# mengxuyiGit/LGM

Measured on AMD Instinct MI355X. Metric: Mpixels/s fwd+bwd Gaussian raster (256^2, 100k gauss, 6 views), higher is better.
Workload: dtype f32

## Files before the change

lgm_amd/csrc/render_common.h:

```cpp
#pragma once
#include <hip/hip_runtime.h>
#include <stdint.h>

#include "common.h"
#include "lgm_render.h"
#include "work_split.h"

namespace lgm {

constexpr int BX = 16, BY = 16, TILE_PIX = BX * BY;
constexpr int NACC = 10;
constexpr int NACC_V = 6, NACC_S = 4;
__host__ __device__ __forceinline__ size_t acc_index(int q, size_t bvN_i, size_t bN_i, size_t BVN) {
    return q < 5 ? bvN_i * NACC_V + q : q < 9 ? BVN * NACC_V + bN_i * NACC_S + (q - 5) : bvN_i * NACC_V + 5;
}
__host__ __device__ inline size_t acc_elems(size_t B, size_t V, size_t N) { return B * V * N * NACC_V + B * N * NACC_S; }
__host__ __device__ inline size_t acc_side_offset(size_t B, size_t V, size_t N) { return (acc_elems(B, V, N) + 1) & ~(size_t)1; }
__host__ __device__ inline int det_flush_limit_log2(int V, int T, bool scene_record) {
    const long long f = scene_record ? (long long)V * T : (long long)T;
    int c = 0;
    while ((1ll << c) < f) c++;
    return 62 - c;
}
constexpr int LDS_HIST_MAX = 8192;
// ... 214 lines not shown
    const float pw = 1.0f / (hom[3] + 0.0000001f);
    const float ppx = hom[0] * pw, ppy = hom[1] * pw;
    xf43(Vw, g[0], g[1], g[2], pv);
    if (pv[2] <= 0.2f) return false;
    const ProjCtx P = make_proj(Vw, g[0], g[1], g[2], d.fx, d.fy, d.tanx, d.tany);
    float a, b, c;
    cov2d(P, c3, a, b, c);
    const float det = a * c - b * b;
    if (det == 0.0f) return false;
    const float det_inv = 1.f / det;
    const float mid = 0.5f * (a + c);
    const float l1 = mid + sqrtf(fmaxf(0.1f, mid * mid - det));
    const float l2 = mid - sqrtf(fmaxf(0.1f, mid * mid - det));
    const float rad = ceilf(3.f * sqrtf(fmaxf(l1, l2)));
    const float px = ndc2pix(ppx, d.W), py = ndc2pix(ppy, d.H);
    const int r = (int)rad;
    const int x0 = min(d.gx, max(0, (int)((px - r) / BX)));
    const int y0 = min(d.gy, max(0, (int)((py - r) / BY)));
    const int x1 = min(d.gx, max(0, (int)((px + r + BX - 1) / BX)));
    const int y1 = min(d.gy, max(0, (int)((py + r + BY - 1) / BY)));
    if ((x1 - x0) * (y1 - y0) == 0) return false;
    o.x = px; o.y = py; o.depth = pv[2];
    o.A = c * det_inv; o.B = -b * det_inv; o.C = a * det_inv;
    o.opacity = g[3];
    o.x0 = x0; o.y0 = y0; o.x1 = x1; o.y1 = y1; o.radius = r;
    const float op = g[3];
    if (d.options & LGM_RENDER_NO_CULL) {
        o.hx = o.hy = 3.0e38f;
        o.tau = 3.0e38f;
        o.cx0 = x0; o.cx1 = x1; o.cy0 = y0; o.cy1 = y1;
        return true;
    }
    if (!(op * 255.0f > 1.0f)) {
        o.hx = o.hy = -1.f;
        o.tau = -1.f;
        o.cx0 = o.cx1 = x0; o.cy0 = o.cy1 = y0;
        return true;
    }
    const float cond = (a + c) * (a + c) * __builtin_amdgcn_rcpf(det);
    if (!(det > 0.f) || !(cond < 4e4f)) {
        o.hx = o.hy = 3.0e38f;
        o.tau = 3.0e38f;
        o.cx0 = x0; o.cx1 = x1; o.cy0 = y0; o.cy1 = y1;
        return true;
    }
    const float tau = (2.0f * 0.6931471805599453f) * __builtin_amdgcn_logf(255.0f * op) * (1.001f + 2e-5f * cond) + 1e-3f;
    o.tau = tau;
    o.hx = sqrtf(tau * fmaxf(a, 0.f));
    o.hy = sqrtf(tau * fmaxf(c, 0.f));
    const float lx = fmaxf(-1.0f, fminf((float)d.gx, (px - o.hx - (BX - 1)) / BX));
    const float hxt = fmaxf(-1.0f, fminf((float)d.gx, (px + o.hx) / BX));
    const float ly = fmaxf(-1.0f, fminf((float)d.gy, (py - o.hy - (BY - 1)) / BY));
    const float hyt = fmaxf(-1.0f, fminf((float)d.gy, (py + o.hy) / BY));
    o.cx0 = max(x0, (int)ceilf(lx));
    o.cx1 = min(x1, (int)floorf(hxt) + 1);
    o.cy0 = max(y0, (int)ceilf(ly));
    o.cy1 = min(y1, (int)floorf(hyt) + 1);
    if (o.cx1 < o.cx0) o.cx1 = o.cx0;
    if (o.cy1 < o.cy0) o.cy1 = o.cy0;
    return true;
}

__device__ __forceinline__ void load_gaussian(const float *__restrict__ src, float g[14]) {
    const float2 *p = reinterpret_cast<const float2 *>(src);
#pragma unroll
    for (int k = 0; k < 7; k++) {
        const float2 v = p[k];
        g[2 * k] = v.x;
        g[2 * k + 1] = v.y;
    }
}

__device__ __forceinline__ void tile_range(int tile, long long slot_stride, const int *__restrict__ tile_start,
                                           const int *__restrict__ tile_count, long long &base, int &n) {
    if (slot_stride >= 0) {
        base = (long long)tile * slot_stride;
        n = tile_count[tile];
    } else {
        base = tile_start[tile];
        n = tile_start[tile + 1] - tile_start[tile];
    }
}

__host__ __device__ __forceinline__ int round8(int x) { return (x + 7) & ~7; }

__device__ __forceinline__ void tile_pixel(int t, int &lx, int &ly) {
    const int w = t >> 6, l = t & 63;
    lx = ((w & 1) << 3) + (l & 7);
    ly = ((w >> 1) << 3) + (l >> 3);
}

int launch_binning(const Dims &d, const float *gaussians, const float *cam_view, const float *cam_view_proj,
                   char *ws, const Layout &L, int *radii_out, long long *stats_out, bool count_only,
                   hipStream_t st);
int launch_render_fwd(const Dims &d, const float *gaussians, const float *bg, float *image, float *depth,
                      float *alpha, char *ws, const Layout &L, hipStream_t st);
int launch_loss_reduce(const Dims &d, char *ws, const Layout &L, hipStream_t st);
int launch_render_bwd(const Dims &d, const float *gaussians, const float *cam_view, const float *cam_view_proj,
                      const float *bg, const float *d_image, const float *d_depth, const float *d_alpha,
                      float *d_gaussians, float *d_means2D, char *ws, const Layout &L, hipStream_t st);

}
```

lgm_amd/csrc/render_raster.hip:

```cpp
#include "cdna4.h"
#include "render_common.h"

#include <type_traits>

namespace lgm {
namespace {

__device__ __forceinline__ unsigned long long lanemask_lt(int lane) { return (1ull << lane) - 1ull; }

#if defined(LGM_BWD_STAMPS) || defined(LGM_FWD_STAMPS)
__device__ __forceinline__ unsigned long long sec_stamp() {
    unsigned long long t;
    __builtin_amdgcn_sched_barrier(0);
    asm volatile("s_memtime %0\n\ts_waitcnt lgkmcnt(0)" : "=s"(t)::"memory");
    __builtin_amdgcn_sched_barrier(0);
    return t;
}
#define SEC_T(v) const unsigned long long v = sec_stamp()
#define SEC_ADD(acc, a, b) acc += (b) - (a)
#else
#define SEC_T(v)
#define SEC_ADD(acc, a, b)
#endif

// ... 121 lines not shown
                                                    const unsigned long long *__restrict__ pairs,
                                                    const float4 *__restrict__ gP, const float4 *__restrict__ gQ,
                                                    const float *__restrict__ gauss,
                                                    const float *__restrict__ bg, float *__restrict__ out_img,
                                                    float *__restrict__ out_depth, float *__restrict__ out_alpha,
                                                    float *__restrict__ final_T, int *__restrict__ n_contrib,
                                                    int *__restrict__ wlast_out,
                                                    unsigned char *__restrict__ cmask, float4 *__restrict__ cfin,
                                                    float *__restrict__ ck, int2 *__restrict__ cklist,
                                                    int *__restrict__ nck, unsigned *__restrict__ ckctr,
                                                    int ck_region, float4 *__restrict__ zero_base,
                                                    long long zero_n16) {
    __shared__ StageT<1, FU> S;
    __shared__ int s_ck[2];
    const int tile = xcd_item(blockIdx.x, d.BV * d.T);
    const int bv = tile / d.T, t = tile - bv * d.T, b = bv / d.V;
    const int tx0 = (t % d.gx) * BX, ty0 = (t / d.gx) * BY;
    const int tid = threadIdx.x, w = tid >> 6, lane = tid & 63;
    int lx, ly;
    tile_pixel(tid, lx, ly);
    const int px = tx0 + lx, py = ty0 + ly;
    const bool inside = px < d.W && py < d.H;
    const float pfx = (float)px, pfy = (float)py;
    long long base;
    int n;
    tile_range(tile, slot_stride, tile_start, tile_count, base, n);
    const unsigned *ids = reinterpret_cast<const unsigned *>(pairs + base);
    const size_t gbase = (size_t)bv * d.N;
    const unsigned long long t_start = __builtin_amdgcn_s_memrealtime();
    init_sentinel(S);
    float Tr = inside ? 1.0f : -1.0f, C0 = 0.f, C1 = 0.f, C2 = 0.f, D = 0.f;
    int last = 0;
    unsigned c_iter = 0, c_list = 0;
    unsigned id_a = tid < n ? ids[tid] : 0u;
    unsigned id_b = TILE_PIX + tid < n ? ids[TILE_PIX + tid] : 0u;
    const int ck_reg = xcd_group(tile, d.BV * d.T);
    const bool det_ck = (d.options & LGM_RENDER_DETERMINISTIC) != 0;
    int ck_slot = -1, ck_written = 0;
#ifdef LGM_FWD_STAMPS
    unsigned long long fs_head = 0, fs_mid = 0, fs_comp = 0;
    const unsigned long long fs_t0 = sec_stamp();
#endif
    for (int b0 = 0, c = 0; b0 < n; b0 += TILE_PIX, c++) {
#ifdef LGM_FWD_STAMPS
        const unsigned long long fs_a = sec_stamp();
#endif
        if (tid == 0) s_ck[c & 1] = ck_slot;
        if (__syncthreads_count(Tr < 0.f) == TILE_PIX) break;
        c_list += min(TILE_PIX, n - b0);
        const int k = b0 + tid;
        StageBuf &B = S.buf[0];
        if (k < n) stage_dma(B, w, id_a, gbase, b, d.N, gP, gQ, gauss);
        vm_wait();
        stage_commit(S, B, tid, k < n, 0u, tx0, ty0, false);
        __syncthreads();
#ifdef LGM_FWD_STAMPS
        const unsigned long long fs_b = sec_stamp();
        fs_head += fs_b - fs_a;
#endif
        if (tid == 0) {
            ck_slot = -1;
            if (b0 + TILE_PIX < n && !det_ck && ((c + 1) & ((1 << d.ck_shift) - 1)) == 0) {
                const unsigned l = atomicAdd(&ckctr[ck_reg], 1u);
                if (l < (unsigned)ck_region) ck_slot = (int)l * 8 + ck_reg;
            }
        }
        if (c >= 1) {
            const int sl = s_ck[c & 1];
            if (sl >= 0) {
                int ctid = tid;
                asm volatile("" : "+v"(ctid));
                float *cp = ck + (size_t)sl * 5 * TILE_PIX + ctid;
                cp[0] = fabsf(Tr);
                cp[TILE_PIX] = C0;
                cp[2 * TILE_PIX] = C1;
                cp[3 * TILE_PIX] = C2;
                cp[4 * TILE_PIX] = D;
                if (tid == 0) {
                    cklist[sl] = make_int2(tile, c >> d.ck_shift);
                    ck_written = c >> d.ck_shift;
                }
            }
        }
        id_a = id_b;
        id_b = k + 2 * TILE_PIX < n ? ids[k + 2 * TILE_PIX] : 0u;
        const int cnt = compact_wave(S, w, lane);
#ifdef LGM_FWD_STAMPS
        const unsigned long long fs_c = sec_stamp();
        fs_mid += fs_c - fs_b;
#endif
        uint2 lraw[FU / 4];
        list_raw<FU>(S, w, 0, lraw);
        for (int kk = 0; kk < cnt; kk += FU) {
            if (__ballot(Tr > 0.f) == 0ull) break;
            c_iter += min(FU, cnt - kk);
            int jj[FU];
            list_decode<FU>(lraw, jj);
            float al[FU];
            float4 cc[FU], Pv[FU], Qv[FU];
#pragma unroll
            for (int u = 0; u < FU; u++) {
                Pv[u] = B.P[jj[u]];
                Qv[u] = B.Q[jj[u]];
                const float4 R = B.R[jj[u]];
                cc[u] = make_float4(R.x, R.y, R.z, 0.f);
            }
            list_raw<FU>(S, w, kk + FU, lraw);
            __builtin_amdgcn_sched_barrier(0);
#pragma unroll
            for (int u = 0; u < FU; u++) {
                const float4 P = Pv[u], Q = Qv[u];
                cc[u].w = Q.w;
                const float dx = P.x - pfx, dy = P.y - pfy;
                const float lp = fmaf(Q.x * dy, dy, fmaf(fmaf(P.w, dy, P.z * dx), dx, Q.y));
                const float e = __builtin_amdgcn_exp2f(lp);
                const float alpha = alpha_cap(e);
                al[u] = (lp > Q.y || e < 1.0f / 255.0f) ? 0.f : alpha;
            }
#pragma unroll
            for (int u = 0; u < FU; u++) {
                const float alpha = al[u];
                const float test_T = Tr * (1 - alpha);
                const bool keep = test_T >= 0.0001f;
                const float aw = keep ? alpha * Tr : 0.f;
                C0 = fmaf(cc[u].x, aw, C0);
                C1 = fmaf(cc[u].y, aw, C1);
                C2 = fmaf(cc[u].z, aw, C2);
                D = fmaf(cc[u].w, aw, D);
                Tr = keep ? test_T : -fabsf(Tr);
                const bool acc = keep && alpha != 0.f;
                last = acc ? b0 + jj[u] + 1 : last;
            }
        }
#ifdef LGM_FWD_STAMPS
        fs_comp += sec_stamp() - fs_c;
#endif
    }
#ifdef LGM_FWD_STAMPS
    if (d.counters && tid == 0) {
        d.counters[8 + 8 * (size_t)tile + 2] = fs_head;
        d.counters[8 + 8 * (size_t)tile + 3] = fs_mid;
        d.counters[8 + 8 * (size_t)tile + 4] = fs_comp;
        d.counters[8 + 8 * (size_t)tile + 5] = sec_stamp() - fs_t0;
    }
#endif
    if (zero_n16 > 0) {
        const long long per = (zero_n16 + gridDim.x - 1) / gridDim.x, z0 = per * blockIdx.x;
        const long long z1 = min(zero_n16, z0 + per);
        for (long long q = z0 + tid; q < z1; q += TILE_PIX) zero_base[q] = make_float4(0.f, 0.f, 0.f, 0.f);
    }
    if (tid == 0) {
        if (ck_slot >= 0) cklist[ck_slot] = make_int2(-1, 0);
        nck[tile] = ck_written;
    }
    {
        const int wl = wave_max_i32(last);
        if (lane == 0) wlast_out[4 * (size_t)tile + w] = wl;
    }
    if (d.counters) {
        if (tid == 0) {
            const unsigned hw_id = __builtin_amdgcn_s_getreg((31 << 11) | 4);
            const unsigned xcc = __builtin_amdgcn_s_getreg((3 << 11) | 20);
            d.counters[8 + 8 * (size_t)tile] = t_start;
            d.counters[8 + 8 * (size_t)tile + 1] = __builtin_amdgcn_s_memrealtime();
            d.counters[8 + 8 * (size_t)tile + 6] = (unsigned long long)(unsigned)n | ((unsigned long long)hw_id << 32);
            d.counters[8 + 8 * (size_t)tile + 7] = (unsigned long long)c_list | ((unsigned long long)c_iter << 32) |
// ... 213 lines not shown
                                                      const float *__restrict__ d_img, const float *__restrict__ d_depth,
                                                      const float *__restrict__ d_alpha,
                                                      const unsigned char *__restrict__ cmask,
                                                      unsigned *__restrict__ det_max, unsigned *__restrict__ det_sat) {
    __shared__ unsigned s_m[4];
    if (blockIdx.x == 0 && threadIdx.x == 0) *det_sat = 0u;
    int lx, ly;
    tile_pixel(threadIdx.x, lx, ly);
    const size_t P = (size_t)d.H * d.W;
    float m = 0.f;
    for (int tile = blockIdx.x; tile < d.BV * d.T; tile += gridDim.x) {
        const int bv = tile / d.T, t = tile - bv * d.T;
        const int px = (t % d.gx) * BX + lx, py = (t / d.gx) * BY + ly;
        const bool inside = px < d.W && py < d.H;
        const size_t pid = inside ? (size_t)d.W * py + px : 0;
        PixelSeed sd;
        pixel_seed<DEPTH, LOSS>(d, inside, bv, P, pid, inside ? final_T[bv * P + pid] : 0.f, bg, cfin, d_img, d_depth,
                                d_alpha, cmask, sd);
        m = fmaxf(m, fmaxf(fmaxf(fabsf(sd.dp0), fabsf(sd.dp1)),
                           fmaxf(fmaxf(fabsf(sd.dp2), fabsf(sd.dpd)), fabsf(sd.dpa))));
    }
    unsigned mb = __float_as_uint(m);
#pragma unroll
    for (int o = 32; o > 0; o >>= 1) mb = max(mb, (unsigned)__shfl_xor((int)mb, o, 64));
    if ((threadIdx.x & 63) == 0) s_m[threadIdx.x >> 6] = mb;
    __syncthreads();
    if (threadIdx.x == 0) {
        mb = max(max(s_m[0], s_m[1]), max(s_m[2], s_m[3]));
        if (mb) atomicMax(det_max + blockIdx.x % DET_SLOTS, mb);
    }
}

template <bool DEPTH, bool LOSS, bool DET>
__global__ __launch_bounds__(256) __attribute__((amdgpu_waves_per_eu(DEPTH ? 2 : 4))) void k_render_bwd(
    Dims d, long long slot_stride, const int *__restrict__ tile_start,
    const int *__restrict__ tile_count, const unsigned long long *__restrict__ pairs, const float4 *__restrict__ gP,
    const float4 *__restrict__ gQ, const float *__restrict__ gauss, const float *__restrict__ bg,
    const float *__restrict__ final_T, const int *__restrict__ n_contrib, const int *__restrict__ wlast_fwd,
    const float4 *__restrict__ cfin, const float *__restrict__ ck, const int2 *__restrict__ cklist,
    const int *__restrict__ nck,
    const unsigned *__restrict__ ckctr, int ck_region, const float *__restrict__ d_img,
    const float *__restrict__ d_depth, const float *__restrict__ d_alpha, const unsigned char *__restrict__ cmask,
    float *__restrict__ accum, const unsigned *__restrict__ det_max, unsigned *__restrict__ det_sat,
    long long item_stamps) {
    constexpr int NV = DEPTH ? NACC : NACC - 1;
    constexpr int CH = BWD_CHUNK, LS = CH + 4;
    __shared__ StageBwd S;
    constexpr int NC = DEPTH ? 4 : 3, NROW = 6 + NC, NROWA = 6 + 2 * NC;
    constexpr int JB = (LS * NROW + 3) & ~3;
    constexpr int SLOT = JB + 64 + CH + 4;
    constexpr int ZSLOT = JB;
    __shared__ __attribute__((aligned(16))) float sAccW[4][SLOT];
    __shared__ __attribute__((aligned(16))) float sWU[4][16 * WU_LD];
    __shared__ __attribute__((aligned(16))) float sO[(NV + 3) * LS];
    __shared__ unsigned sId[CH];
    __shared__ int s_ndl[2];

    const int M = d.BV * d.T, Mp = round8(M);
    int tile, c = 0, slot = -1;
    if ((int)blockIdx.x < M) {
        tile = xcd_item(blockIdx.x, M);
    } else {
        if ((int)blockIdx.x < Mp) return;
        slot = (int)blockIdx.x - Mp;
        if ((int)(slot >> 3) >= (int)ckctr[slot & 7]) return;
        const int2 e = cklist[slot];
        if (e.x < 0) return;
        tile = e.x;
        c = e.y;
    }
    const int bv = tile / d.T, t = tile - bv * d.T, b = bv / d.V;
    const int tx0 = (t % d.gx) * BX, ty0 = (t / d.gx) * BY;
    const int tid = threadIdx.x, w = tid >> 6, lane = tid & 63;
    int lx, ly;
    tile_pixel(tid, lx, ly);
    const int px = tx0 + lx, py = ty0 + ly;
    const bool inside = px < d.W && py < d.H;
    const float pfx = (float)px, pfy = (float)py;
    long long base;
    int n;
    tile_range(tile, slot_stride, tile_start, tile_count, base, n);
    const unsigned *ids = reinterpret_cast<const unsigned *>(pairs + base);
    const bool stager = w == 0;
    const int s0e = (c * TILE_PIX) << d.ck_shift;
    unsigned id_cur = stager && s0e + lane < n ? ids[s0e + lane] : 0u;
    if (stager && s0e + lane < n) stage_dma(S.buf[0], 0, id_cur, (size_t)bv * d.N, b, d.N, gP, gQ, gauss);
    unsigned id_next = stager && s0e + BWD_CHUNK + lane < n ? ids[s0e + BWD_CHUNK + lane] : 0u;
    const size_t P = (size_t)d.H * d.W;
    const size_t pid = inside ? (size_t)d.W * py + px : 0;
    const float T_final = inside ? final_T[bv * P + pid] : 0.f;
    const int last = inside ? n_contrib[bv * P + pid] : 0;
    float ckT = 1.0f, ck1 = 0.f, ck2 = 0.f, ck3 = 0.f, ck4 = 0.f;
    if (slot >= 0) {
        const float *cp = ck + (size_t)slot * 5 * TILE_PIX;
        ckT = cp[tid];
        ck1 = cp[TILE_PIX + tid];
        ck2 = cp[2 * TILE_PIX + tid];
        ck3 = cp[3 * TILE_PIX + tid];
        if (DEPTH) ck4 = cp[4 * TILE_PIX + tid];
    }
    PixelSeed sd;
    pixel_seed<DEPTH, LOSS>(d, inside, bv, P, pid, T_final, bg, cfin, d_img, d_depth, d_alpha, cmask, sd);
    const float dp0 = sd.dp0, dp1 = sd.dp1, dp2 = sd.dp2, dpd = sd.dpd, dpa = sd.dpa;
    const float4 cf = sd.cf;
    float Tr = 1.0f, Dup = 0.f;
    if (slot >= 0) {
        Tr = ckT;
        Dup = fmaf(ck1, dp0, fmaf(ck2, dp1, ck3 * dp2));
        if (DEPTH) Dup = fmaf(ck4, dpd, Dup);
    }
    init_sentinel(S);
    const int4 wl4 = reinterpret_cast<const int4 *>(wlast_fwd)[tile];
    const int wlast = w == 0 ? wl4.x : w == 1 ? wl4.y : w == 2 ? wl4.z : wl4.w;
    const int nlist = min(n, max(max(wl4.x, wl4.y), max(wl4.z, wl4.w)));
    const int s0 = (c * TILE_PIX) << d.ck_shift;
    if (s0 >= nlist) {
        vm_wait();
        return;
    }
    const int s1 = (c + 1 <= nck[tile]) ? min(nlist, s0 + (TILE_PIX << d.ck_shift)) : nlist;
    if (s0 >= s1) {
        vm_wait();
        return;
    }
    const unsigned long long t_item = d.counters ? __builtin_amdgcn_s_memrealtime() : 0ull;
#ifdef LGM_BWD_STAMPS
    unsigned long long sec[8] = {0, 0, 0, 0, 0, 0, 0, 0};
    SEC_T(ts_item);
#endif
    const float bg_dot = bg[0] * dp0 + bg[1] * dp1 + bg[2] * dp2;
    float cdpf = fmaf(cf.x, dp0, fmaf(cf.y, dp1, cf.z * dp2));
    if (DEPTH) cdpf = fmaf(cf.w, dpd, cdpf);
    const float DK = cdpf - (dpa - bg_dot) * T_final;
    float Erem = DK - Dup;
    const float ddelx_dx = 0.5f * d.W, ddely_dy = 0.5f * d.H;
    const int det_s = DET ? det_seed_shift(det_max) : 0;
    const float det_lim_v = ldexpf(1.f, d.det_lim_log2 ? d.det_lim_log2 : det_flush_limit_log2(d.V, d.T, false));
    const float det_lim_s = ldexpf(1.f, d.det_lim_log2 ? d.det_lim_log2 : det_flush_limit_log2(d.V, d.T, true));
    const size_t gbase = (size_t)bv * d.N;
    const int ql = lane & 15, qk = lane >> 4;
    const float cxT = (float)tx0 + 7.5f, cyT = (float)ty0 + 7.5f;
    int mrow[4];
#pragma unroll
    for (int rr = 0; rr < 4; rr++) {
        int row = -1;
        if (ql < MB) {
            if (4 * qk + rr <= 5) row = 4 * qk + rr;
        } else if (rr < 2) {
            const int a = 4 * qk + 2 * rr;
            if (a >= 6 && a < NROWA) row = 6 + (a - 6) / 2;
        }
        mrow[rr] = row >= 0 ? row * LS : JB + lane;
    }
    float *myAcc = sAccW[w];
    float *myWU = sWU[w];
    const int lane_x = lane ^ 8;
    myWU[lane] = dp0;
    myWU[64 + lane] = dp1;
    myWU[128 + lane] = dp2;
    myWU[192 + lane] = dpd;
    __builtin_amdgcn_fence(__ATOMIC_ACQ_REL, "wavefront");
    bf16x8 Ah[2];
    {
        const float fx0 = (float)((w & 1) << 3) - 7.5f, fy0 = (float)((w >> 1) << 3) - 7.5f;
        const bool isdp = ql >= 6 && ql < NROWA, islo = isdp && ((ql - 6) & 1);
        const int qd = isdp ? (ql - 6) >> 1 : 0;
#pragma unroll
        for (int t2 = 0; t2 < 2; t2++) {
            const float fy = fy0 + (float)(4 * t2 + qk);
            const float ca = ql == 0 ? 1.f : ql == 1 ? fx0 : ql == 2 ? fy : ql == 3 ? fx0 * fx0
                           : ql == 4 ? fx0 * fy : ql == 5 ? fy * fy : 0.f;
            const float cb = ql == 1 ? 1.f : ql == 3 ? 2.f * fx0 : ql == 4 ? fy : 0.f;
            const float cc2 = ql == 3 ? 1.f : 0.f;
            const float4 *src = reinterpret_cast<const float4 *>(myWU + qd * 64 + 32 * t2 + 8 * qk);
            const float4 d0 = src[0], d1 = src[1];
            const float dv[8] = {d0.x, d0.y, d0.z, d0.w, d1.x, d1.y, d1.z, d1.w};
#pragma unroll
            for (int j = 0; j < 8; j++) {
                const float geo = fmaf(fmaf(cc2, (float)j, cb), (float)j, ca);
                const __bf16 dh = (__bf16)dv[j];
                const float dlo = dv[j] - (float)dh;
                Ah[t2][j] = ql <= 5 ? (__bf16)geo : !isdp ? (__bf16)0.f : islo ? (__bf16)dlo : dh;
            }
        }
    }
    __builtin_amdgcn_fence(__ATOMIC_ACQ_REL, "wavefront");
    int myj = 0;
    auto read_batch = [&](float (&xs)[2][8]) {
#pragma unroll
        for (int t2 = 0; t2 < 2; t2++) {
            const float *row = myWU + ql * WU_LD;
            const int p0 = 32 * t2 + 8 * qk, sw = wu_swz(ql);
            const float4 x0 = *reinterpret_cast<const float4 *>(row + (p0 ^ sw));
            const float4 x1 = *reinterpret_cast<const float4 *>(row + ((p0 + 4) ^ sw));
            xs[t2][0] = x0.x; xs[t2][1] = x0.y; xs[t2][2] = x0.z; xs[t2][3] = x0.w;
            xs[t2][4] = x1.x; xs[t2][5] = x1.y; xs[t2][6] = x1.z; xs[t2][7] = x1.w;
        }
    };
    auto mfma_batch = [&](const float (&xs)[2][8], int col) {
        f32x4 a2[2];
#pragma unroll
        for (int t2 = 0; t2 < 2; t2++) {
            bf16x8 bh, bl;
#pragma unroll
            for (int j = 0; j < 8; j += 2) {
                const bf16x2v hp = __builtin_convertvector((f32x2v){xs[t2][j], xs[t2][j + 1]}, bf16x2v);
                const unsigned hb = __builtin_bit_cast(unsigned, hp);
                const float h0 = __builtin_bit_cast(float, hb << 16), h1 = __builtin_bit_cast(float, hb & 0xffff0000u);
                const bf16x2v lp = __builtin_convertvector((f32x2v){xs[t2][j] - h0, xs[t2][j + 1] - h1}, bf16x2v);
                bh[j] = hp[0];
                bh[j + 1] = hp[1];
                bl[j] = lp[0];
                bl[j + 1] = lp[1];
            }
            f32x4 cacc = {0.f, 0.f, 0.f, 0.f};
            cacc = __builtin_amdgcn_mfma_f32_16x16x32_bf16(Ah[t2], bh, cacc, 0, 0, 0);
            cacc = __builtin_amdgcn_mfma_f32_16x16x32_bf16(Ah[t2], bl, cacc, 0, 0, 0);
            a2[t2] = cacc;
        }
        const f32x4 acc = a2[0] + a2[1];
        const bool ucol = ql >= MB;
        const float v0 = ucol ? acc[0] + acc[1] : acc[0], v1 = ucol ? acc[2] + acc[3] : acc[1];
        myAcc[mrow[0] + col] = v0;
        myAcc[mrow[1] + col] = v1;
        myAcc[mrow[2] + col] = acc[2];
        myAcc[mrow[3] + col] = acc[3];
    };

    vm_wait();
    __syncthreads();
    int cur = 0;
#ifdef LGM_BWD_STAMPS
    SEC_T(ts_loop);
    SEC_ADD(sec[0], ts_item, ts_loop);
#endif
    for (int b0 = s0, ci = 0; b0 < s1; b0 += CH, cur ^= 1, ci++) {
#ifdef LGM_BWD_STAMPS
        SEC_T(ts_c0b);
#endif
        auto &B = S.buf[cur];
        if (stager) reinterpret_cast<unsigned *>(&B.R[lane])[3] = id_cur;
        if (!DET && tid == 0) s_ndl[ci & 1] = 0;
        {
            float4 *z = reinterpret_cast<float4 *>(myAcc);
            for (int q = lane; q < ZSLOT / 4; q += 64) z[q] = make_float4(0.f, 0.f, 0.f, 0.f);
        }
        int cnt;
        {
            bool hit = false;
            if (b0 + lane < s1 && lane < wlast - b0) {
                const float4 p = B.P[lane], q = B.Q[lane];
                const float qx = (float)(tx0 + ((w & 1) << 3)), qy = (float)(ty0 + ((w >> 1) << 3));
                hit = rec_hits_rect(p, q, qx, qx + 7.0f, qy, qy + 7.0f);
            }
            const unsigned long long bal = __ballot(hit);
            if (hit) S.list[w][__popcll(bal & lanemask_lt(lane))] = (unsigned short)lane;
            cnt = __popcll(bal);
            constexpr int PAD = (int)(sizeof(S.list[0]) / sizeof(S.list[0][0])) - CH;
            if (lane < PAD) S.list[w][cnt + lane] = (unsigned short)CH;
        }
        if (stager && b0 + lane + CH < s1) stage_dma(S.buf[cur ^ 1], 0, id_next, gbase, b, d.N, gP, gQ, gauss);
        id_cur = id_next;
        id_next = stager && b0 + lane + 2 * CH < s1 ? ids[b0 + lane + 2 * CH] : 0u;
        static_assert(MB == 8, "one batch = two 4-entry list words");
#ifdef LGM_BWD_STAMPS
        SEC_T(ts_c1);
        SEC_ADD(sec[2], ts_c0b, ts_c1);
#endif
        const int lastrel = last - b0;
        uint2 lraw[2];
        list_raw<MB>(S, w, 0, lraw);
        auto eval_batch = [&](int kk) {
            int jj8[MB];
            list_decode<MB>(lraw, jj8);
            myj = S.list[w][kk + (lane & (MB - 1))];
            list_raw<MB>(S, w, kk + MB, lraw);
#pragma unroll
            for (int h = 0; h < 2; h++) {
                if (h == 1 && kk + 4 >= cnt) break;
                float al[4], Gw[4];
                float4 cc[4], Pv[4], Qv[4];
#pragma unroll
                for (int u = 0; u < 4; u++) {
                    const int j = jj8[4 * h + u];
                    Pv[u] = B.P[j];
                    Qv[u] = B.Q[j];
                    const float4 Rj = B.R[j];
                    cc[u] = make_float4(Rj.x, Rj.y, Rj.z, 0.f);
                }
                __builtin_amdgcn_sched_barrier(0);
#pragma unroll
                for (int u = 0; u < 4; u++) {
                    const bool before_last = jj8[4 * h + u] < lastrel;
                    const float4 Pj = Pv[u], Q = Qv[u];
                    cc[u].w = Q.w;
                    const float dx = Pj.x - pfx, dy = Pj.y - pfy;
                    const float lp = fmaf(Q.x * dy, dy, fmaf(fmaf(Pj.w, dy, Pj.z * dx), dx, Q.y));
                    const float e = __builtin_amdgcn_exp2f(lp);
                    const bool ok = before_last && lp <= Q.y && e >= 1.0f / 255.0f;
                    Gw[u] = ok ? e : 0.f;
                    al[u] = alpha_cap(Gw[u]);
                }
#pragma unroll
                for (int u = 0; u < 4; u++) {
                    const float alpha = al[u];
                    const float4 cu = cc[u];
                    float cdp = fmaf(cu.x, dp0, fmaf(cu.y, dp1, cu.z * dp2));
                    if (DEPTH) cdp = fmaf(cu.w, dpd, cdp);
                    const float aT = alpha * Tr;
                    const float om = 1.f - alpha;
                    const float inv = __builtin_amdgcn_rcpf(om);
                    Erem = fmaf(-aT, cdp, Erem);
                    const float dL_dalpha = fmaf(Tr, cdp, -Erem * inv);
                    Tr = Tr - aT;
                    myWU[(4 * h + u) * WU_LD + (h == 1 ? lane_x : lane)] = Gw[u] * dL_dalpha;
                    myWU[(MB + 4 * h + u) * WU_LD + (h == 0 ? lane_x : lane)] = aT;
                }
            }
        };
        if (cnt > 0) {
            eval_batch(0);
            for (int kk = 0; kk < cnt; kk += MB) {
                __builtin_amdgcn_fence(__ATOMIC_ACQ_REL, "wavefront");
                float xs[2][8];
                read_batch(xs);
                const int col = myj;
                __builtin_amdgcn_fence(__ATOMIC_ACQ_REL, "wavefront");
                if (kk + MB < cnt) eval_batch(kk + MB);
                mfma_batch(xs, col);
            }
            __builtin_amdgcn_fence(__ATOMIC_ACQ_REL, "wavefront");
        }
#ifdef LGM_BWD_STAMPS
        SEC_T(ts_c2);
        SEC_ADD(sec[3], ts_c1, ts_c2);
#endif
        __syncthreads();
        float *o = sO;
        if (w < 3 && b0 + lane < s1) {
            const int j = lane;
            auto msum = [&](int row) {
                float v = 0.f;
#pragma unroll
                for (int ww = 0; ww < 4; ww++) v += sAccW[ww][row * LS + j];
                return v;
            };
            if (w == 2) {
#pragma unroll
                for (int qq = 6; qq < NV; qq++) {
                    float v = 0.f;
#pragma unroll
                    for (int ww = 0; ww < 4; ww++) v += sAccW[ww][qq * LS + j];
                    o[qq * LS + j] = DET ? ldexpf(v, det_s) : v;
                }
            } else {
                const float4 Pj = B.P[j];
                const float4 Qj = B.Q[j];
                float cA, cB, cC, op;
                rec_conic(Pj, Qj, cA, cB, cC, op);
                const float xg = Pj.x - cxT, yg = Pj.y - cyT;
                const float q0 = msum(0), q1 = msum(1), q2 = msum(2);
                DetNorm nm;
                if (DET) nm = det_norm(Pj.z, Pj.w, Qj.x, d.W, d.H);
                if (w == 0) {
                    sId[j] = reinterpret_cast<const unsigned *>(&B.R[j])[3];
                    const float Sx = fmaf(xg, q0, -q1), Sy = fmaf(yg, q0, -q2);
                    float p0 = -ddelx_dx * (cA * Sx + cB * Sy);
                    float p1 = -ddely_dy * (cC * Sy + cB * Sx);
                    float p5 = op > 0.f ? q0 / op : 0.f;
                    if (DET) {
                        p0 = ldexpf(p0, det_s + nm.k[0]);
                        p1 = ldexpf(p1, det_s + nm.k[1]);
                        p5 = ldexpf(p5, det_s);
                    }
                    o[0 * LS + j] = p0;
                    o[1 * LS + j] = p1;
                    o[5 * LS + j] = p5;
                } else {
                    const float q3 = msum(3), q4 = msum(4), q5 = msum(5);
                    const float Sxx = fmaf(xg, fmaf(xg, q0, -2.f * q1), q3);
                    const float Sxy = fmaf(xg, fmaf(yg, q0, -q2), fmaf(-yg, q1, q4));
                    const float Syy = fmaf(yg, fmaf(yg, q0, -2.f * q2), q5);
                    float pc[3] = {-0.5f * Sxx, -0.5f * Sxy, -0.5f * Syy};
                    if (DET) {
#pragma unroll
                        for (int qq = 0; qq < 3; qq++) pc[qq] = ldexpf(pc[qq], det_s + nm.k[2 + qq]);
                    }
                    const bool ndl = !DET && rec_needle(Pj.z, Pj.w, Qj.x);
#pragma unroll
                    for (int qq = 0; qq < 3; qq++) {
                        o[(2 + qq) * LS + j] = ndl ? 0.f : pc[qq];
                        if (!DET) o[(NV + qq) * LS + j] = ndl ? pc[qq] : 0.f;
                    }
                    if (ndl) s_ndl[ci & 1] = 1;
                }
            }
        }
#ifdef LGM_BWD_STAMPS
        SEC_T(ts_c3);
        SEC_ADD(sec[4], ts_c2, ts_c3);
#endif
        vm_wait();
#ifdef LGM_BWD_STAMPS
        SEC_T(ts_c3a);
        SEC_ADD(sec[5], ts_c3, ts_c3a);
#endif
        __syncthreads();
#ifdef LGM_BWD_STAMPS
        SEC_T(ts_c3b);
        SEC_ADD(sec[6], ts_c3a, ts_c3b);
#endif
        constexpr int FT = 256, FQ = NACC;
        {
        int ft = tid;
        asm volatile("" : "+v"(ft));
#pragma unroll
        for (int it = 0; it < (CH * FQ + FT - 1) / FT; it++) {
            const int f = it * FT + ft;
            const int j = f / FQ, q = f - j * FQ;
            if (q < NV && j < CH && b0 + j < s1) {
                const float a = o[q * LS + j];
                const unsigned gid = sId[j];
                const size_t ai = acc_index(q, gbase + gid, (size_t)b * d.N + gid, (size_t)d.BV * d.N);
                if (a != 0.f) {
                    if (DET) {
                        if (!(fabsf(a) <= (q >= 5 && q < 9 ? det_lim_s : det_lim_v))) atomicAdd(det_sat, 1u);
                        atomicAdd(reinterpret_cast<unsigned long long *>(accum) + ai,
                                  (unsigned long long)__float2ll_rn(fminf(fmaxf(a, -9.0e18f), 9.0e18f)));
                    } else {
                        atomicAdd(accum + ai, a);
                    }
                }
            }
        }
        if (!DET && s_ndl[ci & 1]) {
            int tt = tid;
            asm volatile("" : "+v"(tt));
            for (; tt < 3 * CH; tt += FT) {
                const int j = tt % CH, c3 = tt / CH;
                const float a = o[(NV + c3) * LS + j];
                if (a != 0.f && b0 + j < s1) {
                    const unsigned gid = sId[j];
                    const size_t so = acc_side_offset(d.B, d.V, d.N) / 2;
                    atomicAdd(reinterpret_cast<double *>(accum) + so + (gbase + gid) * 3 + c3, (double)a);
                }
            }
        }
        }
#ifdef LGM_BWD_STAMPS
        SEC_T(ts_c4);
        SEC_ADD(sec[7], ts_c3b, ts_c4);
#endif
    }
#ifdef LGM_BWD_STAMPS
    if (d.counters && lane == 0)
#pragma unroll
        for (int q = 0; q < 8; q++) atomicAdd(&d.counters[q], sec[q]);
#endif
    if (d.counters && tid == 0) {
        unsigned long long *o = d.counters + item_stamps + 4 * (size_t)blockIdx.x;
        o[0] = t_item;
        o[1] = __builtin_amdgcn_s_memrealtime();
        o[2] = (unsigned long long)(s1 - s0) | ((unsigned long long)c << 20) | ((unsigned long long)tile << 40);
        o[3] = (unsigned long long)__builtin_amdgcn_s_getreg((3 << 11) | 20) |
               ((unsigned long long)__builtin_amdgcn_s_getreg((31 << 11) | 4) << 8);
    }
}

__device__ __forceinline__ ProjCtx make_proj_bwd(const float *Vw, float mx, float my, float mz, float fx, float fy,
                                                 float tanx, float tany) {
    ProjCtx P;
    P.t[0] = Vw[0] * mx + Vw[4] * my + Vw[8] * mz + Vw[12];
    P.t[1] = Vw[1] * mx + Vw[5] * my + Vw[9] * mz + Vw[13];
    P.t[2] = Vw[2] * mx + Vw[6] * my + Vw[10] * mz + Vw[14];
    const float limx = 1.3f * tanx, limy = 1.3f * tany, rtz = __builtin_amdgcn_rcpf(P.t[2]);
    const float txtz = P.t[0] * rtz, tytz = P.t[1] * rtz;
    P.t[0] = fminf(limx, fmaxf(-limx, txtz)) * P.t[2];
    P.t[1] = fminf(limy, fmaxf(-limy, tytz)) * P.t[2];
    P.xmul = (txtz < -limx || txtz > limx) ? 0.f : 1.f;
    P.ymul = (tytz < -limy || tytz > limy) ? 0.f : 1.f;
    const float J00 = fx * rtz, J02 = -(fx * P.t[0]) * rtz * rtz;
    const float J11 = fy * rtz, J12 = -(fy * P.t[1]) * rtz * rtz;
#pragma unroll
    for (int r = 0; r < 3; r++) {
        P.T0[r] = Vw[4 * r + 0] * J00 + Vw[4 * r + 2] * J02;
        P.T1[r] = Vw[4 * r + 1] * J11 + Vw[4 * r + 2] * J12;
    }
    return P;
}
__device__ __forceinline__ void cov2d_bwd(const ProjCtx &P, const float c3[6], float &a, float &b, float &c) {
    const float S[3][3] = {{c3[0], c3[1], c3[2]}, {c3[1], c3[3], c3[4]}, {c3[2], c3[4], c3[5]}};
    float s0[3], s1[3];
#pragma unroll
    for (int k = 0; k < 3; k++) {
        s0[k] = S[k][0] * P.T0[0] + S[k][1] * P.T0[1] + S[k][2] * P.T0[2];
        s1[k] = S[k][0] * P.T1[0] + S[k][1] * P.T1[1] + S[k][2] * P.T1[2];
    }
    a = P.T0[0] * s0[0] + P.T0[1] * s0[1] + P.T0[2] * s0[2] + 0.3f;
    b = s1[0] * P.T0[0] + s1[1] * P.T0[1] + s1[2] * P.T0[2];
    c = P.T1[0] * s1[0] + P.T1[1] * s1[1] + P.T1[2] * s1[2] + 0.3f;
}

constexpr int PRE_MAXV = 32;
template <bool LDSV>
__global__ __launch_bounds__(256) void k_preproc_bwd(Dims d, const float *__restrict__ gauss,
                                                     const float *__restrict__ views,
                                                     const float *__restrict__ projs, const uint2 *__restrict__ rects,
                                                     float *__restrict__ accum, float *__restrict__ d_gauss,
                                                     float *__restrict__ d_means2D, const float4 *__restrict__ gP,
                                                     const float4 *__restrict__ gQ,
                                                     const unsigned *__restrict__ det_max,
                                                     const unsigned *__restrict__ det_sat) {
    const bool det = (d.options & LGM_RENDER_DETERMINISTIC) != 0;
    const int det_s = det ? det_seed_shift(det_max) : 0;
    const bool det_bad = det && *det_sat != 0u;
    const int i = blockIdx.x * blockDim.x + threadIdx.x;
    const int b = blockIdx.y;
    const size_t g_diag = (size_t)blockIdx.y * gridDim.x + blockIdx.x;
    const bool stamp = d.counters && threadIdx.x == 0 && g_diag < (size_t)d.BV * d.T;
    if (stamp) d.counters[8 + 8 * g_diag + 2] = __builtin_amdgcn_s_memrealtime();
    const bool live = i < d.N;
    const float fx = d.fx, fy = d.fy, mod = d.mod;
    uint2 r_nx = make_uint2(0u, 0u);
    float2 acc_nx[NACC_V / 2];
    auto load_view = [&](int v) {
        const size_t k = ((size_t)b * d.V + v) * d.N + i;
        r_nx = rects[k];
        if (!det) {
            const float2 *acc2 = reinterpret_cast<const float2 *>(accum + k * NACC_V);
#pragma unroll
            for (int q = 0; q < NACC_V / 2; q++) acc_nx[q] = acc2[q];
        }
    };
    float g[14];
    const size_t ks = (size_t)d.BV * d.N * NACC_V + ((size_t)b * d.N + i) * NACC_S;
    float4 acc_s = make_float4(0.f, 0.f, 0.f, 0.f);
    if (LDSV && live) {
        load_gaussian(gauss + ((size_t)b * d.N + i) * 14, g);
        if (d.V > 0) load_view(0);
        if (!det) acc_s = *reinterpret_cast<const float4 *>(accum + ks);
    }
    __shared__ float s_vp[LDSV ? PRE_MAXV : 1][32];
    if constexpr (LDSV) {
        for (int t = threadIdx.x; t < 32 * d.V; t += blockDim.x) {
            const int v = t >> 5, e = t & 31, bv = b * d.V + v;
            s_vp[v][e] = e < 16 ? views[16 * bv + e] : projs[16 * bv + e - 16];
        }
        __syncthreads();
// ... 240 lines not shown
```

Measured before the change: 2634.

## Reuse forward per-wave hit masks to compact backward gaussian list

The forward raster now writes each tile's per-wave (8x8 quadrant) hit mask byte into spare space after the pair ids. The backward kernel reads these masks, keeps only entries that hit some wave before its last contributor, compacts them into a shared-memory ring queue, and stages only those gaussians. This drops the per-entry rectangle test and skips chunks of non-contributing gaussians, cutting DMA staging and evaluation work. The cost is extra forward global stores, mask loads, queue bookkeeping with ballots, and an assumption that the pairs buffer has room past the ids for the masks.

```diff
diff --git a/lgm_amd/csrc/render_common.h b/lgm_amd/csrc/render_common.h
--- a/lgm_amd/csrc/render_common.h
+++ b/lgm_amd/csrc/render_common.h
@@ -320,6 +320,10 @@
     }
 }
 
+__device__ __forceinline__ unsigned char *tile_masks(const unsigned long long *pairs, long long base, int n) {
+    return reinterpret_cast<unsigned char *>(const_cast<unsigned long long *>(pairs + base)) + 4 * (size_t)n;
+}
+
 __host__ __device__ __forceinline__ int round8(int x) { return (x + 7) & ~7; }
 
 __device__ __forceinline__ void tile_pixel(int t, int &lx, int &ly) {
diff --git a/lgm_amd/csrc/render_raster.hip b/lgm_amd/csrc/render_raster.hip
--- a/lgm_amd/csrc/render_raster.hip
+++ b/lgm_amd/csrc/render_raster.hip
@@ -227,6 +227,11 @@
                 }
             }
         }
+        if (k < n) {
+            int mtid = tid;
+            asm volatile("" : "+v"(mtid));
+            tile_masks(pairs, base, n)[b0 + mtid] = S.mask[mtid];
+        }
         id_a = id_b;
         id_b = k + 2 * TILE_PIX < n ? ids[k + 2 * TILE_PIX] : 0u;
         const int cnt = compact_wave(S, w, lane);
@@ -606,10 +611,25 @@
     tile_range(tile, slot_stride, tile_start, tile_count, base, n);
     const unsigned *ids = reinterpret_cast<const unsigned *>(pairs + base);
     const bool stager = w == 0;
-    const int s0e = (c * TILE_PIX) << d.ck_shift;
-    unsigned id_cur = stager && s0e + lane < n ? ids[s0e + lane] : 0u;
-    if (stager && s0e + lane < n) stage_dma(S.buf[0], 0, id_cur, (size_t)bv * d.N, b, d.N, gP, gQ, gauss);
-    unsigned id_next = stager && s0e + BWD_CHUNK + lane < n ? ids[s0e + BWD_CHUNK + lane] : 0u;
+    constexpr int DW = 2 * 64;
+    constexpr int QN = 2 * BWD_CHUNK + DW;
+    static_assert((QN & (QN - 1)) == 0, "the queue is a ring indexed modulo a power of two");
+    __shared__ unsigned sQ[QN];
+    const int s0 = (c * TILE_PIX) << d.ck_shift;
+    const size_t gbase = (size_t)bv * d.N;
+    unsigned id_cur = stager && s0 + lane < n ? ids[s0 + lane] : 0u;
+    if (stager && s0 + lane < n) stage_dma(S.buf[0], 0, id_cur, gbase, b, d.N, gP, gQ, gauss);
+    const unsigned char *masks = tile_masks(pairs, base, n);
+    const unsigned mrow0 = stager && s0 + lane < n ? masks[s0 + lane] : 0u;
+    auto load_window = [&](int wp) -> unsigned {
+        int ml = lane;
+        asm volatile("" : "+v"(ml));
+        const int p = wp + 2 * ml;
+        return stager && p < n ? (unsigned)*reinterpret_cast<const unsigned short *>(masks + (unsigned)p) : 0u;
+    };
+    const unsigned mwin0 = load_window(s0 + BWD_CHUNK), mwin1 = load_window(s0 + BWD_CHUNK + DW);
+    const int4 wl4 = reinterpret_cast<const int4 *>(wlast_fwd)[tile];
+    const int nck_t = nck[tile];
     const size_t P = (size_t)d.H * d.W;
     const size_t pid = inside ? (size_t)d.W * py + px : 0;
     const float T_final = inside ? final_T[bv * P + pid] : 0.f;
@@ -634,18 +654,50 @@
         if (DEPTH) Dup = fmaf(ck4, dpd, Dup);
     }
     init_sentinel(S);
-    const int4 wl4 = reinterpret_cast<const int4 *>(wlast_fwd)[tile];
-    const int wlast = w == 0 ? wl4.x : w == 1 ? wl4.y : w == 2 ? wl4.z : wl4.w;
     const int nlist = min(n, max(max(wl4.x, wl4.y), max(wl4.z, wl4.w)));
-    const int s0 = (c * TILE_PIX) << d.ck_shift;
     if (s0 >= nlist) {
         vm_wait();
         return;
     }
-    const int s1 = (c + 1 <= nck[tile]) ? min(nlist, s0 + (TILE_PIX << d.ck_shift)) : nlist;
+    const int s1 = (c + 1 <= nck_t) ? min(nlist, s0 + (TILE_PIX << d.ck_shift)) : nlist;
     if (s0 >= s1) {
         vm_wait();
         return;
+    }
+    int qh = 0, qn = 0, wpos = s0 + CH;
+    unsigned mwin = mwin1;
+    auto wave_bits = [&](int p) -> unsigned {
+        return p < s1 ? (unsigned)(p < wl4.x) | ((unsigned)(p < wl4.y) << 1) | ((unsigned)(p < wl4.z) << 2) |
+                            ((unsigned)(p < wl4.w) << 3)
+                      : 0u;
+    };
+    auto append_window = [&](unsigned m2) {
+        const int p = wpos + 2 * lane;
+        const unsigned e0 = m2 & wave_bits(p), e1 = (m2 >> 8) & wave_bits(p + 1);
+        const unsigned long long h0 = __ballot(e0 != 0u), h1 = __ballot(e1 != 0u), lt = lanemask_lt(lane);
+        const int at = qh + qn + __popcll(h0 & lt) + __popcll(h1 & lt);
+        if (e0) sQ[at & (QN - 1)] = ((unsigned)p << 4) | e0;
+        if (e1) sQ[(at + (e0 ? 1 : 0)) & (QN - 1)] = ((unsigned)(p + 1) << 4) | e1;
+        qn += __popcll(h0) + __popcll(h1);
+        wpos += DW;
+    };
+    auto fill_queue = [&]() {
+        while (qn < 2 * CH && wpos < s1) {
+            const unsigned m2 = mwin;
+            mwin = load_window(wpos + DW);
+            append_window(m2);
+        }
+        __builtin_amdgcn_fence(__ATOMIC_ACQ_REL, "wavefront");
+    };
+    auto queue_word = [&](int k) -> unsigned { return k < qn ? sQ[(qh + k) & (QN - 1)] : 0u; };
+    unsigned id_next = 0u;
+    if (stager) {
+        const unsigned e0 = mrow0 & wave_bits(s0 + lane);
+        reinterpret_cast<unsigned *>(&S.buf[0].R[lane])[3] = e0 ? ((unsigned)(s0 + lane) << 4) | e0 : 0u;
+        append_window(mwin0);
+        fill_queue();
+        const unsigned e1 = queue_word(lane);
+        id_next = e1 ? ids[e1 >> 4] : 0u;
     }
     const unsigned long long t_item = d.counters ? __builtin_amdgcn_s_memrealtime() : 0ull;
 #ifdef LGM_BWD_STAMPS
@@ -657,11 +709,9 @@
     if (DEPTH) cdpf = fmaf(cf.w, dpd, cdpf);
     const float DK = cdpf - (dpa - bg_dot) * T_final;
     float Erem = DK - Dup;
-    const float ddelx_dx = 0.5f * d.W, ddely_dy = 0.5f * d.H;
     const int det_s = DET ? det_seed_shift(det_max) : 0;
     const float det_lim_v = ldexpf(1.f, d.det_lim_log2 ? d.det_lim_log2 : det_flush_limit_log2(d.V, d.T, false));
     const float det_lim_s = ldexpf(1.f, d.det_lim_log2 ? d.det_lim_log2 : det_flush_limit_log2(d.V, d.T, true));
-    const size_t gbase = (size_t)bv * d.N;
     const int ql = lane & 15, qk = lane >> 4;
     const float cxT = (float)tx0 + 7.5f, cyT = (float)ty0 + 7.5f;
     int mrow[4];
@@ -753,17 +803,22 @@
 
     vm_wait();
     __syncthreads();
-    int cur = 0;
+    int cur = 0, ci = 0;
+    const int last4 = last << 4;
 #ifdef LGM_BWD_STAMPS
     SEC_T(ts_loop);
     SEC_ADD(sec[0], ts_item, ts_loop);
 #endif
-    for (int b0 = s0, ci = 0; b0 < s1; b0 += CH, cur ^= 1, ci++) {
+    for (;; cur ^= 1, ci++) {
 #ifdef LGM_BWD_STAMPS
         SEC_T(ts_c0b);
 #endif
         auto &B = S.buf[cur];
-        if (stager) reinterpret_cast<unsigned *>(&B.R[lane])[3] = id_cur;
+        const unsigned rowq = reinterpret_cast<const unsigned *>(&B.R[lane])[3];
+        const unsigned long long anyrow = __ballot((rowq & 15u) != 0u);
+        const int rows = anyrow ? 64 - __builtin_clzll(anyrow) : 0;
+        if (rows == 0 && ci > 0) break;
+        if (stager) reinterpret_cast<unsigned *>(&B.Q[lane])[2] = id_cur;
         if (!DET && tid == 0) s_ndl[ci & 1] = 0;
         {
             float4 *z = reinterpret_cast<float4 *>(myAcc);
@@ -771,27 +826,30 @@
         }
         int cnt;
         {
-            bool hit = false;
-            if (b0 + lane < s1 && lane < wlast - b0) {
-                const float4 p = B.P[lane], q = B.Q[lane];
-                const float qx = (float)(tx0 + ((w & 1) << 3)), qy = (float)(ty0 + ((w >> 1) << 3));
-                hit = rec_hits_rect(p, q, qx, qx + 7.0f, qy, qy + 7.0f);
-            }
+            const bool hit = (rowq >> w) & 1u;
             const unsigned long long bal = __ballot(hit);
             if (hit) S.list[w][__popcll(bal & lanemask_lt(lane))] = (unsigned short)lane;
             cnt = __popcll(bal);
             constexpr int PAD = (int)(sizeof(S.list[0]) / sizeof(S.list[0][0])) - CH;
             if (lane < PAD) S.list[w][cnt + lane] = (unsigned short)CH;
         }
-        if (stager && b0 + lane + CH < s1) stage_dma(S.buf[cur ^ 1], 0, id_next, gbase, b, d.N, gP, gQ, gauss);
-        id_cur = id_next;
-        id_next = stager && b0 + lane + 2 * CH < s1 ? ids[b0 + lane + 2 * CH] : 0u;
+        if (stager) {
+            fill_queue();
+            const unsigned e1 = queue_word(lane);
+            reinterpret_cast<unsigned *>(&S.buf[cur ^ 1].R[lane])[3] = e1;
+            if (e1) stage_dma(S.buf[cur ^ 1], 0, id_next, gbase, b, d.N, gP, gQ, gauss);
+            const unsigned e2 = queue_word(CH + lane);
+            const int popped = min(qn, CH);
+            qh = (qh + popped) & (QN - 1);
+            qn -= popped;
+            id_cur = id_next;
+            id_next = e2 ? ids[e2 >> 4] : 0u;
+        }
         static_assert(MB == 8, "one batch = two 4-entry list words");
 #ifdef LGM_BWD_STAMPS
         SEC_T(ts_c1);
         SEC_ADD(sec[2], ts_c0b, ts_c1);
 #endif
-        const int lastrel = last - b0;
         uint2 lraw[2];
         list_raw<MB>(S, w, 0, lraw);
         auto eval_batch = [&](int kk) {
@@ -809,13 +867,12 @@
                     const int j = jj8[4 * h + u];
                     Pv[u] = B.P[j];
                     Qv[u] = B.Q[j];
-                    const float4 Rj = B.R[j];
-                    cc[u] = make_float4(Rj.x, Rj.y, Rj.z, 0.f);
+                    cc[u] = B.R[j];
                 }
                 __builtin_amdgcn_sched_barrier(0);
 #pragma unroll
                 for (int u = 0; u < 4; u++) {
-                    const bool before_last = jj8[4 * h + u] < lastrel;
+                    const bool before_last = __float_as_int(cc[u].w) < last4;
                     const float4 Pj = Pv[u], Q = Qv[u];
                     cc[u].w = Q.w;
                     const float dx = Pj.x - pfx, dy = Pj.y - pfy;
@@ -861,7 +918,7 @@
 #endif
         __syncthreads();
         float *o = sO;
-        if (w < 3 && b0 + lane < s1) {
+        if (w < 3 && lane < rows) {
             const int j = lane;
             auto msum = [&](int row) {
                 float v = 0.f;
@@ -885,9 +942,12 @@
                 const float xg = Pj.x - cxT, yg = Pj.y - cyT;
                 const float q0 = msum(0), q1 = msum(1), q2 = msum(2);
                 DetNorm nm;
-                if (DET) nm = det_norm(Pj.z, Pj.w, Qj.x, d.W, d.H);
+                int cW = d.W, cH = d.H;
+                asm volatile("" : "+s"(cW), "+s"(cH));
+                const float ddelx_dx = 0.5f * cW, ddely_dy = 0.5f * cH;
+                if (DET) nm = det_norm(Pj.z, Pj.w, Qj.x, cW, cH);
                 if (w == 0) {
-                    sId[j] = reinterpret_cast<const unsigned *>(&B.R[j])[3];
+                    sId[j] = __float_as_uint(Qj.z);
                     const float Sx = fmaf(xg, q0, -q1), Sy = fmaf(yg, q0, -q2);
                     float p0 = -ddelx_dx * (cA * Sx + cB * Sy);
                     float p1 = -ddely_dy * (cC * Sy + cB * Sx);
@@ -942,7 +1002,7 @@
         for (int it = 0; it < (CH * FQ + FT - 1) / FT; it++) {
             const int f = it * FT + ft;
             const int j = f / FQ, q = f - j * FQ;
-            if (q < NV && j < CH && b0 + j < s1) {
+            if (q < NV && j < rows) {
                 const float a = o[q * LS + j];
                 const unsigned gid = sId[j];
                 const size_t ai = acc_index(q, gbase + gid, (size_t)b * d.N + gid, (size_t)d.BV * d.N);
@@ -963,7 +1023,7 @@
             for (; tt < 3 * CH; tt += FT) {
                 const int j = tt % CH, c3 = tt / CH;
                 const float a = o[(NV + c3) * LS + j];
-                if (a != 0.f && b0 + j < s1) {
+                if (a != 0.f && j < rows) {
                     const unsigned gid = sId[j];
                     const size_t so = acc_side_offset(d.B, d.V, d.N) / 2;
                     atomicAdd(reinterpret_cast<double *>(accum) + so + (gbase + gid) * 3 + c3, (double)a);
@@ -987,7 +1047,8 @@
         o[1] = __builtin_amdgcn_s_memrealtime();
         o[2] = (unsigned long long)(s1 - s0) | ((unsigned long long)c << 20) | ((unsigned long long)tile << 40);
         o[3] = (unsigned long long)__builtin_amdgcn_s_getreg((3 << 11) | 20) |
-               ((unsigned long long)__builtin_amdgcn_s_getreg((31 << 11) | 4) << 8);
+               ((unsigned long long)__builtin_amdgcn_s_getreg((31 << 11) | 4) << 8) |
+               ((unsigned long long)ci << 40);
     }
 }
 
```

Result: no change. 2649 (median of 6 runs) (+0.5%).
